# topling/toplingdb

Measured on NVIDIA H100. Metric: compaction_input_kv_MB_per_s, higher is better.
Workload: dtype u8

## Files before the change

### toplingdb_b200/csrc/api.cu

```cuda
#include <cuda_runtime.h>
#include <stdio.h>
#include <stdlib.h>
#include <string.h>

#include <algorithm>
#include <map>
#include <memory>
#include <mutex>
#include <unordered_map>
#include <string>
#include <thread>
#include <vector>

#include "../../include/b200c.h"
#include "inflate_rules.h"
#include "kernels.h"
#include "range_plan.h"
#include "scan.cuh"
#include "sst_host.h"

using namespace b200c;

namespace {

// ... 185 lines not shown
  const char* name;
  cudaEvent_t a, b;
  float us;
};

}

struct b200c_job {
  b200c_params p;
  std::vector<uint64_t> snapshots, fct;
  std::string cf_name, db_id, db_session_id, db_host_id;
  std::vector<Input> inputs;
  std::vector<Output> outputs;
  b200c_stats stats;
  bool ran = false;
  int stage_done = 0;
  int sms = 132;
  cudaStream_t st = nullptr;
  cudaStream_t st2 = nullptr;
  cudaStream_t st_up = nullptr;
  cudaEvent_t ev[5] = {nullptr, nullptr, nullptr, nullptr, nullptr};
  cudaEvent_t evx[4] = {nullptr, nullptr, nullptr, nullptr};
  DevBuf files_d, blk_off, blk_size, blk_state, scan_tmp, run_start, small;
  DevBuf dec[4], mrg[4], splits, tile_state, snaps_d;
  DevBuf esz, eshared, tstat, nxt, disk, rows, tstate, grows, gstate, gflag, gsync, idx_contrib, idx_contrib_off, blocks, files_rec, idx_esz, idx_eoff, idx_sep, out_buf, out_base_d;
  uint64_t n_total = 0, n_out = 0, nblk_in = 0, nblocks_out = 0;
  uint32_t nfiles_out = 0, nruns = 0;
  DevBuf bloom_contrib, bloom_contrib_off;
  DevBuf bloom_hashes;
  DevBuf kv_arena, kv_offs, kv_klens;
  DevBuf run_bounds, run_first_d;
  std::vector<uint64_t> run_start_h;
  HostBuf host_out;
  std::vector<GpKey> gp_small, gp_large;
  std::vector<uint64_t> gp_size;
  std::vector<uint8_t> gp_same;
  DevBuf gp_keys_d, gp_ranks_d, gp_size_d, gp_same_d, gp_cuts_d;
  BoundKey range_lo{}, range_hi{};
  DevBuf clip_d;
  DevBuf cslot, cslot_off, arena;
  std::vector<cudaEvent_t> range_events;
  std::vector<std::string> range_bounds;
  cudaEvent_t wait_ev = nullptr;
  DevBuf vfiles_d, vrun_start;
  HostBuf pin_small, pin_tails, pin_rd, pin_up;
  size_t pin_up_used = 0;
  std::vector<KernelTime> ktimes;
// ... 760 lines not shown
    j->kt_end();
    launches++;
    uint64_t hc[kSmallSlots];
    int rc = read_small(j, small, hc, nullptr, nullptr);
    if (rc) return rc;
    rc = map_dev_err((uint32_t)hc[kSlotErr]);
    if (rc) return rc;
    N_in = hc[kSlotClip];
    range_value_bytes = hc[kSlotClip + 1];
    if (N_in > n_decoded) return fail(B200C_ERR_CUDA, "internal: clipped entry count exceeds the input");
    runs = RunBounds{j->clip_d.as<uint64_t>(), j->clip_d.as<uint64_t>() + K};
    j->stats.num_input_records = N_in;
  }
  return run_merge_encode(j, until, decc, runs, n_decoded, N_in, clipped, range_value_bytes, small, err, launches);
}

int run_merge_encode(b200c_job* j, int until, KeyCols decc, RunBounds runs, uint64_t n_decoded, uint64_t N, bool clipped,
                     uint64_t range_value_bytes, uint64_t* small, uint32_t* err, uint64_t launches) {
  const b200c_params& P = j->p;
  cudaStream_t st = j->st;
  const size_t k = j->nruns;
  const uint64_t mtiles = (N + kMergeNominal - 1) / kMergeNominal;
  CU(j->splits.reserve(8 * (mtiles + 1) * k));
  CU(j->tile_state.reserve(8 * (mtiles + 1)));
  CU(cudaMemsetAsync(j->tile_state.p, 0, 8 * (mtiles + 1), st));
  CU(j->snaps_d.reserve(8 * (P.num_snapshots + 1)));
  if (P.num_snapshots)
    if (int rc = upload_small(j, j->snaps_d.p, j->snapshots.data(), 8 * P.num_snapshots)) return rc;
  CU(j->mrg[0].reserve(16 * (N + 1)));
  CU(j->mrg[1].reserve(8 * (N + 1)));
  CU(j->mrg[2].reserve(8 * (N + 1)));
  CU(j->mrg[3].reserve(4 * (N + 1)));
  CU(j->esz.reserve(4 * (N + 1)));
  CU(j->eshared.reserve(N + 1));
  CU(j->tstat.reserve(sizeof(TileStat) * (mtiles + 2)));
  KeyColsMut mrg{j->mrg[0].as<ulonglong2>(), j->mrg[1].as<uint64_t>(), j->mrg[2].as<uint64_t>(), j->mrg[3].as<uint32_t>()};
  MergeParams mp;
  mp.nruns = (uint32_t)k;
  mp.bottommost = P.bottommost_level != 0;
  mp.nsnapshots = P.num_snapshots;
  mp.snapshots = j->snaps_d.as<uint64_t>();
  mp.earliest_snapshot = P.num_snapshots ? j->snapshots[0] : kMaxSeq;
  mp.filter = P.compaction_filter;
  mp.ttl = P.ttl;
  mp.now = P.ttl_now;
  mp.write_conflict_snapshot = P.earliest_write_conflict_snapshot != 0 && P.earliest_write_conflict_snapshot < kMaxSeq;
  MergeCounters* counters = reinterpret_cast<MergeCounters*>(small + kSlotCounters);
  EncodeWork W;
  memset(&W, 0, sizeof W);
  W.esz = j->esz.as<uint32_t>();
  W.eshared = j->eshared.as<uint8_t>();
  W.tstat = j->tstat.as<TileStat>();
  W.min_s1 = reinterpret_cast<uint32_t*>(small + kSlotMinS1);
  W.totals = small + kSlotTotals;
  if (N) {
    j->kt_begin("merge.partition");
    launch_merge_partition(decc, runs, (uint32_t)k, N, mtiles, j->splits.as<uint64_t>(), err, j->sms, st);
    j->kt_end();
    const MergeSizes msz{W.esz, W.eshared, W.tstat, W.min_s1};
    W.tprefix = j->tile_state.as<unsigned long long>();
    W.nstat = mtiles;
    j->kt_begin("merge.tiles");
    launch_merge_tiles(decc, runs, mp, N, mtiles, j->splits.as<uint64_t>(),
                       j->tile_state.as<unsigned long long>(), reinterpret_cast<uint32_t*>(small + kSlotTicket), mrg, counters, msz, err, st);
    j->kt_end();
    j->kt_begin("merge.sizes_fix");
    launch_merge_sizes_fix(KeyCols{mrg.pfx, mrg.tr, mrg.vref, mrg.meta, 0}, j->tile_state.as<unsigned long long>(), mtiles, msz, st);
    j->kt_end();
    launches += 3;
  }
  CU(cudaEventRecord(j->ev[2], st));
  KeyCols mcols{mrg.pfx, mrg.tr, mrg.vref, mrg.meta, 0};
  uint64_t h[kSmallSlots];
  {
    int rc = read_small(j, small, h, nullptr, nullptr);
    if (rc) return rc;
    rc = map_dev_err((uint32_t)h[kSlotErr]);
    if (rc) return rc;
  }
  if (clipped ? h[kSlotTotalIn] > n_decoded : h[kSlotTotalIn] != n_decoded)
    return fail(B200C_ERR_CORRUPTION, "decoded entry count differs from rocksdb.num.entries");
  MergeCounters mc;
  memcpy(&mc, h + kSlotCounters, sizeof mc);
  const uint64_t n_out = mc.n_out;
  j->n_out = n_out;
  mcols.n = n_out;
// ... 413 lines not shown
  Output& o = j->outputs[i];
  if (cap < o.meta.file_size) return fail(B200C_ERR_INVALID_ARGUMENT, "destination too small");
  if (j->p.output_mem == B200C_MEM_HOST) {
    memcpy(dst, j->host_out.p + o.host_off, o.meta.file_size);
    return B200C_OK;
  }
  CU(cudaSetDevice(j->p.device));
  CU(cudaMemcpy(dst, j->out_buf.as<uint8_t>() + o.dev_off, o.meta.file_size, cudaMemcpyDefault));
  return B200C_OK;
}
int b200c_job_get_stats(const b200c_job* j, b200c_stats* s) {
  if (!j || !s) return fail(B200C_ERR_INVALID_ARGUMENT, "null argument");
  *s = j->stats;
  return B200C_OK;
}
void b200c_job_destroy(b200c_job* j) {
  if (!j) return;
  cudaSetDevice(j->p.device);
  if (j->st) cudaStreamSynchronize(j->st);
  if (j->st2) cudaStreamSynchronize(j->st2);
  if (j->st_up) cudaStreamSynchronize(j->st_up);
  DevBuf* all[] = {&j->files_d, &j->blk_off, &j->blk_size, &j->blk_state, &j->scan_tmp, &j->run_start, &j->run_bounds, &j->run_first_d, &j->kv_arena, &j->kv_offs, &j->kv_klens, &j->bloom_contrib, &j->bloom_contrib_off, &j->bloom_hashes, &j->small,
                   &j->dec[0], &j->dec[1], &j->dec[2], &j->dec[3], &j->mrg[0], &j->mrg[1], &j->mrg[2], &j->mrg[3], &j->splits,
                   &j->tile_state, &j->snaps_d, &j->esz, &j->eshared, &j->tstat, &j->nxt, &j->disk, &j->rows, &j->tstate, &j->grows, &j->gstate, &j->gflag, &j->gsync, &j->idx_contrib, &j->idx_contrib_off, &j->blocks,
                   &j->files_rec, &j->idx_esz, &j->idx_eoff, &j->idx_sep, &j->out_buf, &j->out_base_d};
  for (DevBuf* b : all) b->release();
  j->gp_keys_d.release();
  j->gp_ranks_d.release();
  j->gp_size_d.release();
  j->gp_same_d.release();
  j->gp_cuts_d.release();
  j->clip_d.release();
  j->vfiles_d.release();
  j->vrun_start.release();
  j->cslot.release();
  j->cslot_off.release();
  j->arena.release();
  for (cudaEvent_t e : j->range_events)
    if (e) cudaEventDestroy(e);
  for (auto& in : j->inputs) {
    in.staged.release();
    in.index_inflated.release();
    if (in.up_ev) cudaEventDestroy(in.up_ev);
  }
  if (j->st_up) cudaStreamDestroy(j->st_up);
  j->host_out.release();
  j->pin_small.release();
// ... 167 lines not shown
```

### toplingdb_b200/csrc/kernels.h

```cpp
#pragma once
#include <cuda_runtime.h>
#include <stdint.h>

#include <atomic>

#include "common.cuh"
#include "gp_rules.h"

namespace b200c {

struct PerDeviceFlag {
  std::atomic<uint64_t> mask{0};
  uint64_t bit_of_current_device() const {
    int d = 0;
    cudaGetDevice(&d);
    return 1ull << (d & 63);
  }
  bool is_set(uint64_t bit) const { return (mask.load(std::memory_order_acquire) & bit) != 0; }
  void set(uint64_t bit) { mask.fetch_or(bit, std::memory_order_release); }
};

struct FileDesc {
  const uint8_t* base;
  uint64_t len;
// ... 46 lines not shown
struct MergeParams {
  uint32_t nruns;
  uint32_t bottommost;
  uint32_t nsnapshots;
  const uint64_t* snapshots;
  uint64_t earliest_snapshot;
  uint32_t filter;
  int32_t ttl;
  int64_t now;
  uint32_t write_conflict_snapshot;
};
struct TileStat {
  uint64_t raw_key, raw_value, deletions, smallest_seq, largest_seq;
};
struct MergeSizes {
  uint32_t* esz;
  uint8_t* eshared;
  TileStat* tstat;
  uint32_t* min_s1;
};
struct MergeCounters {
  unsigned long long n_out, n_input_deletions, n_hidden, n_obsolete, raw_key_bytes, raw_value_bytes, n_silent, n_user_drop;
};
struct RunBounds {
  const uint64_t* begin;
  const uint64_t* end;
};
void launch_clip_runs(KeyCols in, RunBounds runs, uint32_t nruns, BoundKey start, uint32_t has_start, BoundKey end,
                      uint32_t has_end, uint64_t* clip, unsigned long long* totals, cudaStream_t st);
void launch_run_bounds(KeyCols in, const uint64_t* file_start, const uint32_t* run_first, uint32_t nruns, uint64_t* bounds, uint32_t* err,
                       cudaStream_t st);
void launch_merge_partition(KeyCols in, RunBounds runs, uint32_t nruns, uint64_t n_total, uint64_t ntiles,
                            uint64_t* splits, uint32_t* err, int sms, cudaStream_t st);
void launch_merge_tiles(KeyCols in, RunBounds runs, MergeParams mp, uint64_t n_total, uint64_t ntiles,
                        const uint64_t* splits, unsigned long long* tile_state, uint32_t* ticket, KeyColsMut out,
                        MergeCounters* counters, MergeSizes ms, uint32_t* err, cudaStream_t st);
void launch_merge_sizes_fix(KeyCols merged, const unsigned long long* tile_state, uint64_t ntiles, MergeSizes ms, cudaStream_t st);

struct GpCut {
  uint64_t entry;
  uint64_t block_bytes;
};
struct EncodeParams {
  uint32_t block_size, block_size_limit , restart_interval;
  uint32_t checksum, format_version, output_level;
  uint64_t max_output_file_size;
  GpCtx gp;
  GpCut* gp_cuts;
  uint32_t* gp_ncuts;
};
using GpKey = BoundKey;
void launch_bloom_count(KeyCols m, uint64_t n, FileRec* files, const uint64_t* nfiles_dev, uint32_t millibits, uint64_t* hashes, int sms, cudaStream_t st);
void launch_bloom_build(const uint64_t* hashes, uint64_t n, const FileRec* files, uint32_t nfiles, uint32_t max_filter_bytes, uint32_t millibits, uint32_t cksum,
                        uint8_t* const* out_base, uint64_t* contrib, const uint64_t* contrib_off, cudaStream_t st);
void launch_gp_ranks(KeyCols m, const GpKey* smallest, const GpKey* largest, uint32_t n, uint64_t* lo, uint64_t* eq, uint64_t* hi,
                     cudaStream_t st);
struct BlockRec {
  uint64_t first_entry;
// ... 83 lines not shown
```

### toplingdb_b200/csrc/merge.cu

```cuda
#include "common.cuh"
#include "group_rules.h"
#include "kernels.h"

namespace b200c {

constexpr int kMT = kMergeTile;
constexpr int kMThreads = 256;
constexpr int kMV = kMT / kMThreads;

__device__ __forceinline__ Key load_key(const KeyCols& c, uint64_t i) {
  Key k;
  ulonglong2 p = c.pfx[i];
  k.hi = p.x;
  k.lo = p.y;
  k.tr = c.tr[i];
  k.ulen = meta_ulen(c.meta[i]);
  return k;
}

__device__ __forceinline__ uint64_t count_before(const KeyCols& c, uint64_t base, uint64_t lo, uint64_t hi, const Key& x,
                                                 bool before_equal) {
  while (lo < hi) {
    uint64_t mid = lo + ((hi - lo) >> 1);
    Key e = load_key(c, base + mid);
    bool precedes = before_equal ? !ikey_less(x, e) : ikey_less(e, x);
    if (precedes) lo = mid + 1;
    else hi = mid;
  }
  return lo;
}

__global__ void __launch_bounds__(128)
merge_partition_kernel(KeyCols in, RunBounds runs, uint32_t nruns, uint64_t n_total, uint64_t ntiles,
                       uint64_t* __restrict__ splits, uint32_t* __restrict__ err) {
  const unsigned lane = threadIdx.x & 31;
  const uint64_t b = (uint64_t)blockIdx.x * (blockDim.x >> 5) + (threadIdx.x >> 5);
  if (b > ntiles) return;
  uint64_t d = b * (uint64_t)kMergeNominal;
  if (d > n_total) d = n_total;
  uint64_t base[2], lo[2], hi[2];
#pragma unroll
  for (int s = 0; s < 2; s++) {
    uint32_t r = lane + 32 * s;
    base[s] = r < nruns ? runs.begin[r] : 0;
    uint64_t n = r < nruns ? runs.end[r] - runs.begin[r] : 0;
    lo[s] = (d == n_total) ? n : 0;
    hi[s] = (d == 0) ? 0 : n;
  }
  for (int guard = 0; guard < 64 * 70; guard++) {
    unsigned long long best = 0;
#pragma unroll
    for (int s = 0; s < 2; s++) {
      unsigned long long wdt = hi[s] - lo[s];
      unsigned long long enc = (wdt << 7) | (unsigned long long)(lane + 32 * s);
      if (wdt && enc > best) best = enc;
    }
#pragma unroll
// ... 18 lines not shown
      sum += c[s];
    }
#pragma unroll
    for (int dd = 16; dd; dd >>= 1) sum += __shfl_xor_sync(0xffffffffu, sum, dd);
    const bool x_before = sum < d;
#pragma unroll
    for (int s = 0; s < 2; s++) {
      uint32_t r = lane + 32 * s;
      if (r >= nruns) continue;
      if (x_before) lo[s] = (r == p) ? m + 1 : c[s];
      else hi[s] = (r == p) ? m : c[s];
    }
  }
  uint64_t tot = lo[0] + lo[1];
#pragma unroll
  for (int dd = 16; dd; dd >>= 1) tot += __shfl_xor_sync(0xffffffffu, tot, dd);
  if (tot != d && lane == 0) atomicOr(err, kErrKeyOrder);
  if (lane == 0 && (*reinterpret_cast<volatile uint32_t*>(err) & (uint32_t)kFlagHasSingleDelete)) atomicOr(err, (uint32_t)kErrGroupTooLong);
#pragma unroll
  for (int s = 0; s < 2; s++) {
    uint32_t r = lane + 32 * s;
    if (r < nruns) splits[b * nruns + r] = lo[s];
  }
}

constexpr uint32_t kPartStride = 64;
struct GroupLanes {
  uint32_t gshift, g, r, sub, gbase, nruns;
};
__device__ __forceinline__ bool entry_precedes(const KeyCols& c, uint64_t i, const Key& x, bool before_equal) {
  const ulonglong2 p = c.pfx[i];
  if (p.x != x.hi) return p.x < x.hi;
  if (p.y != x.lo) return p.y < x.lo;
  const uint32_t ul = meta_ulen(c.meta[i]);
  if (ul != x.ulen) return ul < x.ulen;
  const uint64_t tr = c.tr[i];
  if (tr != x.tr) return tr > x.tr;
  return before_equal;
}
__device__ __forceinline__ void msel_grouped(const KeyCols& in, const GroupLanes& L, uint64_t base, uint64_t stride, uint64_t d, uint64_t& lo,
                                             uint64_t& hi) {
  const uint32_t g = L.g, r = L.r, sub = L.sub, gbase = L.gbase, gshift = L.gshift;
  for (int guard = 0; guard < 64 * 70; guard++) {
    const unsigned long long wdt = hi - lo;
    unsigned long long best = wdt ? ((wdt << 7) | (unsigned long long)r) : 0;
#pragma unroll
// ... 28 lines not shown
      const uint32_t cp = __popc((bal >> gbase) & ((1u << g) - 1u));
      const uint32_t nvalid = w == 0 ? 0 : (w <= g ? (uint32_t)w : g);
      const uint64_t below = __shfl_sync(0xffffffffu, pos, (int)(gbase + (cp ? cp - 1 : 0)));
      const uint64_t above = __shfl_sync(0xffffffffu, pos, (int)(gbase + (cp < g ? cp : g - 1)));
      if (w > 0) {
        if (cp) clo = below + 1;
        if (cp < nvalid) chi = above;
        else if (w <= g) chi = clo;
      }
    }
    const uint64_t c = clo;
    uint64_t sum = sub == 0 ? c : 0;
#pragma unroll
    for (int dd = 16; dd; dd >>= 1) sum += __shfl_xor_sync(0xffffffffu, sum, dd);
    const bool x_before = sum < d;
    if (r < L.nruns) {
      if (x_before) lo = (r == p) ? m + 1 : c;
      else hi = (r == p) ? m : c;
    }
  }
}
__global__ void __launch_bounds__(128, 12)
merge_partition_grouped_kernel(KeyCols in, RunBounds runs, uint32_t nruns, uint32_t gshift, uint64_t n_total,
                               uint64_t ntiles, uint64_t* __restrict__ splits, uint32_t* __restrict__ err, uint32_t chunk) {
  const unsigned lane = threadIdx.x & 31;
  const uint64_t b0 = ((uint64_t)blockIdx.x * (blockDim.x >> 5) + (threadIdx.x >> 5)) * chunk;
  if (b0 > ntiles) return;
  GroupLanes L;
  L.gshift = gshift;
  L.g = 1u << gshift;
  L.r = lane >> gshift;
  L.sub = lane & (L.g - 1);
  L.gbase = L.r << gshift;
  L.nruns = nruns;
  const uint32_t r = L.r, sub = L.sub;
  const uint64_t base = r < nruns ? runs.begin[r] : 0;
  const uint64_t nrun = r < nruns ? runs.end[r] - runs.begin[r] : 0;
  uint64_t prev_lo = 0, prev_d = 0;
  const bool sd_mode = (*reinterpret_cast<volatile uint32_t*>(err) & (uint32_t)kFlagHasSingleDelete) != 0;
  for (uint32_t c = 0; c < chunk; c++) {
    const uint64_t b = b0 + c;
    if (b > ntiles) break;
    uint64_t d = b * (uint64_t)kMergeNominal;
    if (d > n_total) d = n_total;
    uint64_t lo = (d == n_total) ? nrun : 0, hi = (d == 0) ? 0 : nrun;
    if (d != 0 && d != n_total) {
      if (c != 0) {
// ... 39 lines not shown
        const bool ohv = __shfl_xor_sync(0xffffffffu, (int)anyh, dd) != 0, otv = __shfl_xor_sync(0xffffffffu, (int)anyt, dd) != 0;
        if (ohv && (!anyh || ukey_cmp(oh.hi, oh.lo, oh.ulen, mh.hi, mh.lo, mh.ulen) < 0)) mh = oh, anyh = true;
        if (otv && (!anyt || ukey_cmp(ot.hi, ot.lo, ot.ulen, mt.hi, mt.lo, mt.ulen) > 0)) mt = ot, anyt = true;
      }
      if (anyh && anyt && ukey_cmp(mh.hi, mh.lo, mh.ulen, mt.hi, mt.lo, mt.ulen) == 0) {
        uint32_t adv = 0;
        if (r < nruns && sub == 0) {
          while (lo < nrun && adv <= (uint32_t)kSdSpill) {
            const ulonglong2 p = in.pfx[base + lo];
            if (p.x != mh.hi || p.y != mh.lo || meta_ulen(in.meta[base + lo]) != mh.ulen) break;
            lo++;
            adv++;
          }
        }
        uint32_t tadv = adv;
#pragma unroll
        for (int dd = 16; dd; dd >>= 1) tadv += __shfl_xor_sync(0xffffffffu, tadv, dd);
        if (tadv > (uint32_t)kSdSpill && lane == 0) atomicOr(err, (uint32_t)kErrGroupTooLong);
        d += tadv;
        lo = __shfl_sync(0xffffffffu, lo, (int)L.gbase);
      }
    }
    if (r < nruns && sub == 0) splits[b * nruns + r] = lo;
    prev_lo = lo;
    prev_d = d;
  }
}

constexpr uint32_t kSnapCache = 16;
struct TileSmem {
  uint64_t hi[kMT], lo[kMT], tr[kMT];
  uint16_t idx[kMT];
  uint8_t ulen[kMT];
  uint8_t verd[kMT];
  uint32_t seg[kMaxRuns + 1];
  uint32_t lst[2][kMaxRuns + 2];
  uint64_t sbeg[kMaxRuns];
  uint64_t snaps[kSnapCache];
  unsigned long long red[8];
  unsigned long long stat[5];
  uint32_t smin, smax;
  uint32_t wsum[40];
  uint64_t base_out;
  uint32_t tile_id, kept_total;
  Key pred;
  uint32_t has_pred;
};

__device__ __forceinline__ Key skey(const TileSmem& s, uint32_t id) {
  Key k;
  k.hi = s.hi[id];
  k.lo = s.lo[id];
  k.tr = s.tr[id];
  k.ulen = s.ulen[id] & 0x3fu;
  return k;
}
__device__ __forceinline__ uint32_t PH(uint32_t e) { return e ^ ((e >> 4) & 15u); }
__device__ __forceinline__ bool tie_less(const TileSmem& s, uint32_t ib, uint32_t ia) {
  const uint64_t lb = s.lo[ib], la = s.lo[ia];
  if (lb != la) return lb < la;
  const uint32_t ub = s.ulen[ib] & 0x3fu, ua = s.ulen[ia] & 0x3fu;
  if (ub != ua) return ub < ua;
  return s.tr[ib] > s.tr[ia];
}
__device__ __forceinline__ bool id_less(const TileSmem& s, uint32_t ib, uint64_t hb, uint32_t ia, uint64_t ha) {
  if (hb != ha) return hb < ha;
  return tie_less(s, ib, ia);
}

struct PairState {
  uint32_t ai, a1, bi, b1, pend;
};
__device__ __noinline__ void init_pair(const TileSmem& s, const uint32_t* lst, uint32_t nlists, uint32_t o, PairState* ps) {
  uint32_t pi = 0;
  for (;;) {
    uint32_t e = 2 * pi + 2 <= nlists ? lst[2 * pi + 2] : lst[nlists];
    if (o < e) break;
    pi++;
  }
  uint32_t a0 = lst[2 * pi];
  uint32_t a1 = lst[2 * pi + 1];
  bool single = 2 * pi + 1 >= nlists;
  uint32_t b1 = single ? a1 : lst[2 * pi + 2];
  ps->pend = b1;
  ps->a1 = a1;
  ps->b1 = b1;
  if (single) {
    ps->ai = o;
    ps->bi = b1;
    return;
  }
  uint32_t diag = o - a0, an = a1 - a0, bn = b1 - a1;
  uint32_t lo = diag > bn ? diag - bn : 0, hi = diag < an ? diag : an;
  while (lo < hi) {
    uint32_t mid = (lo + hi) >> 1;
    const uint32_t ia = s.idx[PH(a0 + mid)], ib = s.idx[PH(a1 + diag - 1 - mid)];
    if (!id_less(s, ib, s.hi[ib], ia, s.hi[ia])) lo = mid + 1;
    else hi = mid;
  }
  ps->ai = a0 + lo;
  ps->bi = a1 + (diag - lo);
}

__device__ __forceinline__ uint64_t stripe_of(const uint64_t* snaps_s, const uint64_t* snaps_g, uint32_t ns, uint64_t seq,
                                              uint64_t* prev) {
  uint32_t lo = 0, hi = ns;
  while (lo < hi) {
    uint32_t mid = (lo + hi) >> 1;
    uint64_t v = mid < kSnapCache ? snaps_s[mid] : snaps_g[mid];
    if (v < seq) lo = mid + 1;
    else hi = mid;
  }
  *prev = lo == 0 ? 0 : (lo - 1 < kSnapCache ? snaps_s[lo - 1] : snaps_g[lo - 1]);
  return lo < ns ? (lo < kSnapCache ? snaps_s[lo] : snaps_g[lo]) : kMaxSeq;
}

__device__ bool oldest_version_at_most(const KeyCols& in, RunBounds runs, uint32_t nruns, uint64_t hi, uint64_t lo,
                                       uint32_t ulen, uint64_t limit) {
  Key x;
  x.hi = hi;
  x.lo = lo;
  x.ulen = ulen;
  x.tr = 0;
  for (uint32_t r = 0; r < nruns; r++) {
// ... 100 lines not shown
        if (s.seg[mid] <= id0) lo = mid;
        else hi = mid;
      }
      gr.filter_removes_newest = mp.filter == 1 ? (s.ulen[id0] & 0x80u) != 0 : filter_removes(mp, in, s.sbeg[lo] + (id0 - s.seg[lo]));
    }
    gr.first_key_of_the_job = 0;
    GroupVerdict vd[kMaxGroup];
    GroupCounters gc{0, 0, 0, 0};
    if (group_walk(gv, n, gr, vd, &gc) != 0) atomicOr(err, (uint32_t)kErrSingleDelContract);
    for (uint32_t i = 0; i < n; i++)
      s.verd[o + i] = (uint8_t)(0x80u | (vd[i].keep ? 1u : 0u) | (vd[i].zero_seq ? 2u : 0u) | ((vd[i].clear_value & 1u) ? 4u : 0u) |
                                (vd[i].out_type != gv[i].type ? 8u : 0u) | ((vd[i].clear_value & kGrSkipped) ? 16u : 0u));
    *w_hidden += gc.drop_hidden;
    *w_obsolete += gc.drop_obsolete;
    *w_userdrop += gc.drop_user;
  }
  __syncthreads();
}

constexpr int kMergeCtasPerSm = 3;
template <bool kSD>
__global__ void __launch_bounds__(kMThreads, kMergeCtasPerSm)
merge_tiles_kernel(KeyCols in, RunBounds runs, MergeParams mp, uint64_t n_total, uint64_t ntiles,
                   const uint64_t* __restrict__ splits, unsigned long long* tile_state, uint32_t* ticket, KeyColsMut out,
                   MergeCounters* counters, MergeSizes ms, uint32_t* __restrict__ err) {
  extern __shared__ __align__(16) uint8_t smem_raw[];
  TileSmem& s = *reinterpret_cast<TileSmem*>(smem_raw);
  const uint32_t t = threadIdx.x, lane = t & 31, w = t >> 5;
  const uint32_t k = mp.nruns;
  if (((*reinterpret_cast<volatile uint32_t*>(err) & (uint32_t)kFlagHasSingleDelete) != 0) != kSD) return;
  if (t == 0) s.tile_id = atomicAdd(ticket, 1u);
  if (t < 8) s.red[t] = 0;
  if (t < 5) s.stat[t] = t == 3 ? ~0ull : 0ull;
  if (t == 0) {
    s.smin = 0xffffffffu;
    s.smax = 0;
  }
  if (t < kSnapCache && t < mp.nsnapshots) s.snaps[t] = mp.snapshots[t];
  __syncthreads();
  const uint64_t tile = s.tile_id;
  if (tile >= ntiles) return;
  Key* cand = reinterpret_cast<Key*>(s.hi);
  uint32_t* cand_ok = reinterpret_cast<uint32_t*>(s.idx);
  if (t < k) {
    const uint64_t s0 = splits[tile * k + t], s1 = splits[(tile + 1) * k + t];
    const uint64_t b0 = runs.begin[t] + s0;
    s.sbeg[t] = b0;
    s.lst[1][t] = (uint32_t)(s1 - s0);
    cand_ok[t] = s0 != 0;
    if (s0 != 0) cand[t] = load_key(in, b0 - 1);
  }
  __syncthreads();
  if (t == 0) {
    uint32_t acc = 0;
    for (uint32_t r = 0; r < k; r++) {
      s.seg[r] = acc;
      s.lst[0][r] = acc;
      acc += s.lst[1][r];
    }
    s.seg[k] = acc;
    s.lst[0][k] = acc;
    if (acc > kMT) {
      atomicOr(err, kErrKeyOrder);
      s.seg[k] = 0;
    }
    s.has_pred = 0;
    for (uint32_t r = 0; r < k; r++) {
      if (!cand_ok[r]) continue;
      const Key e = cand[r];
      if (!s.has_pred || ikey_less(s.pred, e)) {
        s.pred = e;
        s.has_pred = 1;
      }
    }
  }
  __syncthreads();
  const uint32_t cnt = s.seg[k];
  bool tile_sd = false;
  {
    ulonglong2 lp[kMV];
    uint64_t ltr[kMV];
    uint32_t lmt[kMV];
    uint32_t lr = 0;
    bool my_sd = false;
#pragma unroll
    for (int j = 0; j < kMV; j++) {
      const uint32_t i = t + j * kMThreads;
      lp[j] = make_ulonglong2(0, 0);
      ltr[j] = 0;
      lmt[j] = 0;
      if (i < cnt) {
        while (i >= s.seg[lr + 1]) lr++;
        const uint64_t src = s.sbeg[lr] + (i - s.seg[lr]);
        lp[j] = in.pfx[src];
        ltr[j] = in.tr[src];
        lmt[j] = in.meta[src];
      }
    }
#pragma unroll
    for (int j = 0; j < kMV; j++) {
      const uint32_t i = t + j * kMThreads;
      if (i < cnt) {
        s.hi[i] = lp[j].x;
        s.lo[i] = lp[j].y;
        s.tr[i] = ltr[j];
        if (kSD) my_sd = my_sd || (ltr[j] & 0xff) == kTypeSingleDeletion;
        s.ulen[i] = (uint8_t)(meta_ulen(lmt[j]) | (meta_vlen(lmt[j]) == 0 ? 0x80u : 0u));
        s.idx[PH(i)] = (uint16_t)i;
      }
    }
    if (kSD) tile_sd = __syncthreads_or(my_sd) != 0;
    else __syncthreads();
  }
  uint32_t nlists = k;
  int cur = 0;
  while (nlists > 1) {
    const uint32_t* lst = s.lst[cur];
    uint16_t rid[kMV];
    const uint32_t o0 = t * kMV;
    PairState ps;
    ps.pend = 0;
    ps.ai = ps.a1 = ps.bi = ps.b1 = 0;
    uint32_t ia = 0, ib = 0;
    uint64_t ha = 0, hb = 0;
    bool va = false, vb = false;
#pragma unroll
    for (int x = 0; x < kMV; x++) {
      uint32_t o = o0 + x;
      rid[x] = 0;
      if (o < cnt) {
        if (o >= ps.pend) {
          init_pair(s, lst, nlists, o, &ps);
          va = ps.ai < ps.a1;
          vb = ps.bi < ps.b1;
          if (va) {
            ia = s.idx[PH(ps.ai)];
            ha = s.hi[ia];
          }
          if (vb) {
            ib = s.idx[PH(ps.bi)];
            hb = s.hi[ib];
          }
        }
        const bool take_a = !vb || (va && !id_less(s, ib, hb, ia, ha));
        rid[x] = (uint16_t)(take_a ? ia : ib);
        if (take_a) {
          ps.ai++;
          va = ps.ai < ps.a1;
          if (va) {
            ia = s.idx[PH(ps.ai)];
            ha = s.hi[ia];
          }
        } else {
          ps.bi++;
          vb = ps.bi < ps.b1;
// ... 167 lines not shown
  uint32_t rank = s.wsum[w] + inc - nkeep;
  const uint32_t kept_total = s.kept_total;
  const unsigned long long kAgg = 1ull << 62, kPre = 2ull << 62, kVal = (1ull << 62) - 1;
  if (t == 0) atomicExch(&tile_state[tile], (tile == 0 ? kPre : kAgg) | kept_total);
#pragma unroll
  for (int x = 0; x < kMV; x++) {
    uint32_t o = t * kMV + x;
    if (o < cnt && ((keep_mask >> (16 + x)) & 1)) {
      c_vbytes += meta_vlen(in.meta[col_of(oid[x])]);
    }
  }
  __syncthreads();
#pragma unroll
  for (int x = 0; x < kMV; x++) {
    if ((keep_mask >> x) & 1) {
      s.idx[PH(rank)] = oid[x];
      s.tr[oid[x]] = otr[x];
      if ((keep_mask >> (24 + x)) & 1) s.ulen[oid[x]] |= 0x40u;
      rank++;
    }
  }
  __syncthreads();
  {
    uint64_t gv[kMV];
    uint32_t gm[kMV];
    uint16_t gp[kMV];
#pragma unroll
    for (int j = 0; j < kMV; j++) {
      const uint32_t i = t + j * kMThreads;
      gv[j] = 0;
      gm[j] = 0;
      gp[j] = 0;
      if (i < kept_total) {
        const uint32_t pos = s.idx[PH(i)];
        const uint64_t src = col_of(pos);
        gp[j] = (uint16_t)pos;
        gv[j] = in.vref[src];
        gm[j] = in.meta[src];
        if (s.ulen[pos] & 0x40u) gm[j] = make_meta(meta_ulen(gm[j]), 0);
      }
    }
    if (w == 0) {
      uint64_t base = 0;
      if (tile != 0) {
        int64_t look = (int64_t)tile - 1;
        while (true) {
          const int64_t idx = look - lane;
          unsigned long long sv = kPre;
          if (idx >= 0) {
            sv = *((volatile unsigned long long*)&tile_state[idx]);
            while ((sv >> 62) == 0) {
              __nanosleep(64);
              sv = *((volatile unsigned long long*)&tile_state[idx]);
            }
          }
          const unsigned pre_mask = __ballot_sync(0xffffffffu, (sv >> 62) == 2);
          const int first_pre = pre_mask ? __ffs(pre_mask) - 1 : 32;
          uint64_t contrib = ((int)lane <= first_pre) ? (sv & kVal) : 0;
#pragma unroll
          for (int dd = 16; dd; dd >>= 1) contrib += __shfl_xor_sync(0xffffffffu, contrib, dd);
          base += contrib;
          if (pre_mask) break;
          look -= 32;
        }
        if (lane == 0) atomicExch(&tile_state[tile], kPre | (base + kept_total));
      }
      if (lane == 0) s.base_out = base;
    }
    __syncthreads();
    const uint64_t base_out = s.base_out;
    uint32_t st_kb = 0, st_nd = 0, mn = 0xffffffffu, mx = 0;
    unsigned long long st_vb = 0, st_smin = ~0ull, st_smax = 0;
#pragma unroll
    for (int j = 0; j < kMV; j++) {
      const uint32_t i = t + j * kMThreads;
      if (i < kept_total) {
        const uint32_t pos = gp[j];
        const uint64_t dst = base_out + i;
        const uint64_t chi = s.hi[pos], clo = s.lo[pos], ctr = s.tr[pos];
        const uint32_t cul = s.ulen[pos] & 0x3fu, vlen = meta_vlen(gm[j]);
        out.pfx[dst] = make_ulonglong2(chi, clo);
        out.tr[dst] = ctr;
        out.vref[dst] = gv[j];
        out.meta[dst] = gm[j];
        if (i > 0) {
          const uint32_t pp = s.idx[PH(i - 1)];
          const uint32_t sh = shared_prefix(chi, clo, cul, ctr, s.hi[pp], s.lo[pp], s.ulen[pp] & 0x3fu, s.tr[pp]);
          const uint32_t s1 = entry_size(sh, cul + 8, vlen);
          ms.esz[dst] = s1;
          ms.eshared[dst] = (uint8_t)sh;
          mn = s1 < mn ? s1 : mn;
          mx = s1 > mx ? s1 : mx;
        }
        st_kb += cul + 8;
        st_vb += vlen;
        st_nd += is_deletion_type((uint32_t)(ctr & 0xff));
        const unsigned long long sq = ctr >> 8;
        st_smin = sq < st_smin ? sq : st_smin;
        st_smax = sq > st_smax ? sq : st_smax;
      }
    }
    const unsigned kb = __reduce_add_sync(0xffffffffu, st_kb), nd = __reduce_add_sync(0xffffffffu, st_nd);
    mn = __reduce_min_sync(0xffffffffu, mn);
    mx = __reduce_max_sync(0xffffffffu, mx);
#pragma unroll
    for (int dd = 16; dd; dd >>= 1) {
// ... 110 lines not shown
}
void launch_clip_runs(KeyCols in, RunBounds runs, uint32_t nruns, BoundKey start, uint32_t has_start, BoundKey end,
                      uint32_t has_end, uint64_t* clip, unsigned long long* totals, cudaStream_t st) {
  if (nruns) clip_runs_kernel<<<dim3(kClipSlices, nruns), 256, 0, st>>>(in, runs, nruns, start, has_start, end, has_end, clip, totals);
}
__global__ void run_bounds_kernel(KeyCols in, const uint64_t* __restrict__ file_start, const uint32_t* __restrict__ run_first, uint32_t nruns,
                                  uint64_t* __restrict__ bounds, uint32_t* __restrict__ err) {
  const uint32_t r = blockIdx.x * blockDim.x + threadIdx.x;
  if (r >= nruns) return;
  const uint32_t f0 = run_first[r], f1 = run_first[r + 1];
  bounds[r] = file_start[f0];
  bounds[nruns + r] = file_start[f1];
  for (uint32_t f = f0 + 1; f < f1; f++) {
    const uint64_t e = file_start[f];
    if (e > file_start[f0] && e < file_start[f1] && !ikey_less(load_key(in, e - 1), load_key(in, e))) atomicOr(err, (uint32_t)kErrKeyOrder);
  }
}
void launch_run_bounds(KeyCols in, const uint64_t* file_start, const uint32_t* run_first, uint32_t nruns, uint64_t* bounds, uint32_t* err,
                       cudaStream_t st) {
  if (nruns) run_bounds_kernel<<<(nruns + 63) / 64, 64, 0, st>>>(in, file_start, run_first, nruns, bounds, err);
}

void launch_merge_partition(KeyCols in, RunBounds runs, uint32_t nruns, uint64_t n_total, uint64_t ntiles,
                            uint64_t* splits, uint32_t* err, int sms, cudaStream_t st) {
  unsigned warps = (unsigned)(ntiles + 1);
  if (nruns <= 16) {
    uint32_t kp2 = 2;
    while (kp2 < nruns) kp2 <<= 1;
    uint32_t gshift = 0;
    while ((kp2 << (gshift + 1)) <= 32) gshift++;
    const unsigned wave = (unsigned)sms * 48u;
    uint32_t chunk = (uint32_t)((warps + wave - 1) / wave);
    if (chunk > 4) chunk = 4;
    if (chunk < 1) chunk = 1;
    const unsigned chunks = (warps + chunk - 1) / chunk;
    merge_partition_grouped_kernel<<<(chunks + 3) / 4, 128, 0, st>>>(in, runs, nruns, gshift, n_total, ntiles, splits, err, chunk);
    return;
  }
  merge_partition_kernel<<<(warps + 3) / 4, 128, 0, st>>>(in, runs, nruns, n_total, ntiles, splits, err);
}
static_assert(sizeof(Key) * kMaxRuns <= sizeof(uint64_t) * kMT && 4 * kMaxRuns <= 2 * kMT, "candidate staging must fit");
static_assert(kMergeCtasPerSm * (sizeof(TileSmem) + 1024) <= 227 * 1024, "merge tile must fit three CTAs per SM");
void launch_merge_tiles(KeyCols in, RunBounds runs, MergeParams mp, uint64_t n_total, uint64_t ntiles,
                        const uint64_t* splits, unsigned long long* tile_state, uint32_t* ticket, KeyColsMut out,
                        MergeCounters* counters, MergeSizes ms, uint32_t* err, cudaStream_t st) {
  if (ntiles == 0) return;
  static PerDeviceFlag attr;
  const uint64_t dev_bit = attr.bit_of_current_device();
  if (!attr.is_set(dev_bit)) {
    cudaFuncSetAttribute(merge_tiles_kernel<false>, cudaFuncAttributeMaxDynamicSharedMemorySize, (int)sizeof(TileSmem));
    cudaFuncSetAttribute(merge_tiles_kernel<true>, cudaFuncAttributeMaxDynamicSharedMemorySize, (int)sizeof(TileSmem));
    attr.set(dev_bit);
  }
  merge_tiles_kernel<false><<<(unsigned)ntiles, kMThreads, sizeof(TileSmem), st>>>(in, runs, mp, n_total, ntiles, splits, tile_state, ticket,
                                                                                   out, counters, ms, err);
  merge_tiles_kernel<true><<<(unsigned)ntiles, kMThreads, sizeof(TileSmem), st>>>(in, runs, mp, n_total, ntiles, splits, tile_state, ticket,
                                                                                  out, counters, ms, err);
}
void launch_merge_sizes_fix(KeyCols merged, const unsigned long long* tile_state, uint64_t ntiles, MergeSizes ms, cudaStream_t st) {
  if (ntiles) merge_sizes_fix_kernel<<<(unsigned)((ntiles + 127) / 128), 128, 0, st>>>(merged, tile_state, ntiles, ms);
}

}
```

Before: 244,100.

## Precompute tile predecessor keys in partition and stage tile inputs via cp.async

The partition kernels now compute each tile's predecessor key with a warp shuffle reduction and store it in a new per-tile buffer. This removes the serial loop over runs that thread 0 ran in every merge tile. Merge tiles load keys, tags and value refs straight into shared memory with cp.async, and value refs are now read from shared memory at output time instead of gathered again from global memory. Pair initialisation is partly inlined. Together these add a vref array to shared memory, which may reduce occupancy, and add extra key loads to the partition kernels.

```diff
diff --git a/toplingdb_b200/csrc/api.cu b/toplingdb_b200/csrc/api.cu
--- a/toplingdb_b200/csrc/api.cu
+++ b/toplingdb_b200/csrc/api.cu
@@ -231,7 +231,7 @@
   cudaEvent_t ev[5] = {nullptr, nullptr, nullptr, nullptr, nullptr};
   cudaEvent_t evx[4] = {nullptr, nullptr, nullptr, nullptr};
   DevBuf files_d, blk_off, blk_size, blk_state, scan_tmp, run_start, small;
-  DevBuf dec[4], mrg[4], splits, tile_state, snaps_d;
+  DevBuf dec[4], mrg[4], splits, preds, tile_state, snaps_d;
   DevBuf esz, eshared, tstat, nxt, disk, rows, tstate, grows, gstate, gflag, gsync, idx_contrib, idx_contrib_off, blocks, files_rec, idx_esz, idx_eoff, idx_sep, out_buf, out_base_d;
   uint64_t n_total = 0, n_out = 0, nblk_in = 0, nblocks_out = 0;
   uint32_t nfiles_out = 0, nruns = 0;
@@ -1038,6 +1038,7 @@
   const size_t k = j->nruns;
   const uint64_t mtiles = (N + kMergeNominal - 1) / kMergeNominal;
   CU(j->splits.reserve(8 * (mtiles + 1) * k));
+  CU(j->preds.reserve(sizeof(TilePred) * (mtiles + 1)));
   CU(j->tile_state.reserve(8 * (mtiles + 1)));
   CU(cudaMemsetAsync(j->tile_state.p, 0, 8 * (mtiles + 1), st));
   CU(j->snaps_d.reserve(8 * (P.num_snapshots + 1)));
@@ -1071,13 +1072,13 @@
   W.totals = small + kSlotTotals;
   if (N) {
     j->kt_begin("merge.partition");
-    launch_merge_partition(decc, runs, (uint32_t)k, N, mtiles, j->splits.as<uint64_t>(), err, j->sms, st);
+    launch_merge_partition(decc, runs, (uint32_t)k, N, mtiles, j->splits.as<uint64_t>(), j->preds.as<TilePred>(), err, j->sms, st);
     j->kt_end();
     const MergeSizes msz{W.esz, W.eshared, W.tstat, W.min_s1};
     W.tprefix = j->tile_state.as<unsigned long long>();
     W.nstat = mtiles;
     j->kt_begin("merge.tiles");
-    launch_merge_tiles(decc, runs, mp, N, mtiles, j->splits.as<uint64_t>(),
+    launch_merge_tiles(decc, runs, mp, N, mtiles, j->splits.as<uint64_t>(), j->preds.as<TilePred>(),
                        j->tile_state.as<unsigned long long>(), reinterpret_cast<uint32_t*>(small + kSlotTicket), mrg, counters, msz, err, st);
     j->kt_end();
     j->kt_begin("merge.sizes_fix");
@@ -1537,7 +1538,7 @@
   if (j->st_up) cudaStreamSynchronize(j->st_up);
   DevBuf* all[] = {&j->files_d, &j->blk_off, &j->blk_size, &j->blk_state, &j->scan_tmp, &j->run_start, &j->run_bounds, &j->run_first_d, &j->kv_arena, &j->kv_offs, &j->kv_klens, &j->bloom_contrib, &j->bloom_contrib_off, &j->bloom_hashes, &j->small,
                    &j->dec[0], &j->dec[1], &j->dec[2], &j->dec[3], &j->mrg[0], &j->mrg[1], &j->mrg[2], &j->mrg[3], &j->splits,
-                   &j->tile_state, &j->snaps_d, &j->esz, &j->eshared, &j->tstat, &j->nxt, &j->disk, &j->rows, &j->tstate, &j->grows, &j->gstate, &j->gflag, &j->gsync, &j->idx_contrib, &j->idx_contrib_off, &j->blocks,
+                   &j->preds, &j->tile_state, &j->snaps_d, &j->esz, &j->eshared, &j->tstat, &j->nxt, &j->disk, &j->rows, &j->tstate, &j->grows, &j->gstate, &j->gflag, &j->gsync, &j->idx_contrib, &j->idx_contrib_off, &j->blocks,
                    &j->files_rec, &j->idx_esz, &j->idx_eoff, &j->idx_sep, &j->out_buf, &j->out_base_d};
   for (DevBuf* b : all) b->release();
   j->gp_keys_d.release();
diff --git a/toplingdb_b200/csrc/kernels.h b/toplingdb_b200/csrc/kernels.h
--- a/toplingdb_b200/csrc/kernels.h
+++ b/toplingdb_b200/csrc/kernels.h
@@ -92,6 +92,11 @@
 struct MergeCounters {
   unsigned long long n_out, n_input_deletions, n_hidden, n_obsolete, raw_key_bytes, raw_value_bytes, n_silent, n_user_drop;
 };
+struct alignas(16) TilePred {
+  uint64_t hi, lo, tr;
+  uint32_t ulen, has;
+};
+static_assert(sizeof(TilePred) == 32, "one 32-byte slot per boundary");
 struct RunBounds {
   const uint64_t* begin;
   const uint64_t* end;
@@ -101,9 +106,9 @@
 void launch_run_bounds(KeyCols in, const uint64_t* file_start, const uint32_t* run_first, uint32_t nruns, uint64_t* bounds, uint32_t* err,
                        cudaStream_t st);
 void launch_merge_partition(KeyCols in, RunBounds runs, uint32_t nruns, uint64_t n_total, uint64_t ntiles,
-                            uint64_t* splits, uint32_t* err, int sms, cudaStream_t st);
+                            uint64_t* splits, TilePred* preds, uint32_t* err, int sms, cudaStream_t st);
 void launch_merge_tiles(KeyCols in, RunBounds runs, MergeParams mp, uint64_t n_total, uint64_t ntiles,
-                        const uint64_t* splits, unsigned long long* tile_state, uint32_t* ticket, KeyColsMut out,
+                        const uint64_t* splits, const TilePred* preds, unsigned long long* tile_state, uint32_t* ticket, KeyColsMut out,
                         MergeCounters* counters, MergeSizes ms, uint32_t* err, cudaStream_t st);
 void launch_merge_sizes_fix(KeyCols merged, const unsigned long long* tile_state, uint64_t ntiles, MergeSizes ms, cudaStream_t st);
 
diff --git a/toplingdb_b200/csrc/merge.cu b/toplingdb_b200/csrc/merge.cu
--- a/toplingdb_b200/csrc/merge.cu
+++ b/toplingdb_b200/csrc/merge.cu
@@ -30,9 +30,21 @@
   return lo;
 }
 
+__device__ __forceinline__ void write_pred(Key m, bool has, TilePred* __restrict__ pred) {
+#pragma unroll
+  for (int dd = 16; dd; dd >>= 1) {
+    Key o;
+    o.hi = __shfl_xor_sync(0xffffffffu, m.hi, dd), o.lo = __shfl_xor_sync(0xffffffffu, m.lo, dd);
+    o.tr = __shfl_xor_sync(0xffffffffu, m.tr, dd), o.ulen = __shfl_xor_sync(0xffffffffu, m.ulen, dd);
+    const bool ohas = __shfl_xor_sync(0xffffffffu, (int)has, dd) != 0;
+    if (ohas && (!has || ikey_less(m, o))) m = o, has = true;
+  }
+  if ((threadIdx.x & 31) == 0) *pred = TilePred{m.hi, m.lo, m.tr, m.ulen, has ? 1u : 0u};
+}
+
 __global__ void __launch_bounds__(128)
 merge_partition_kernel(KeyCols in, RunBounds runs, uint32_t nruns, uint64_t n_total, uint64_t ntiles,
-                       uint64_t* __restrict__ splits, uint32_t* __restrict__ err) {
+                       uint64_t* __restrict__ splits, TilePred* __restrict__ preds, uint32_t* __restrict__ err) {
   const unsigned lane = threadIdx.x & 31;
   const uint64_t b = (uint64_t)blockIdx.x * (blockDim.x >> 5) + (threadIdx.x >> 5);
   if (b > ntiles) return;
@@ -97,6 +109,16 @@
     uint32_t r = lane + 32 * s;
     if (r < nruns) splits[b * nruns + r] = lo[s];
   }
+  Key e[2];
+  bool has[2];
+#pragma unroll
+  for (int s = 0; s < 2; s++) {
+    has[s] = lane + 32 * s < nruns && lo[s] > 0;
+    e[s] = Key{0, 0, 0, 0};
+    if (has[s]) e[s] = load_key(in, base[s] + lo[s] - 1);
+  }
+  if (has[1] && (!has[0] || ikey_less(e[0], e[1]))) e[0] = e[1], has[0] = true;
+  write_pred(e[0], has[0], preds + b);
 }
 
 constexpr uint32_t kPartStride = 64;
@@ -171,7 +193,8 @@
 }
 __global__ void __launch_bounds__(128, 12)
 merge_partition_grouped_kernel(KeyCols in, RunBounds runs, uint32_t nruns, uint32_t gshift, uint64_t n_total,
-                               uint64_t ntiles, uint64_t* __restrict__ splits, uint32_t* __restrict__ err, uint32_t chunk) {
+                               uint64_t ntiles, uint64_t* __restrict__ splits, TilePred* __restrict__ preds, uint32_t* __restrict__ err,
+                               uint32_t chunk) {
   const unsigned lane = threadIdx.x & 31;
   const uint64_t b0 = ((uint64_t)blockIdx.x * (blockDim.x >> 5) + (threadIdx.x >> 5)) * chunk;
   if (b0 > ntiles) return;
@@ -257,6 +280,10 @@
       }
     }
     if (r < nruns && sub == 0) splits[b * nruns + r] = lo;
+    const bool has = r < nruns && sub == 0 && lo > 0;
+    Key e{0, 0, 0, 0};
+    if (has) e = load_key(in, base + lo - 1);
+    write_pred(e, has, preds + b);
     prev_lo = lo;
     prev_d = d;
   }
@@ -265,6 +292,7 @@
 constexpr uint32_t kSnapCache = 16;
 struct TileSmem {
   uint64_t hi[kMT], lo[kMT], tr[kMT];
+  uint64_t vref[kMT];
   uint16_t idx[kMT];
   uint8_t ulen[kMT];
   uint8_t verd[kMT];
@@ -282,6 +310,11 @@
   uint32_t has_pred;
 };
 
+__device__ __forceinline__ void cp_async8(void* smem, const void* gmem) {
+  asm volatile("cp.async.ca.shared.global [%0], [%1], 8;" ::"r"((uint32_t)__cvta_generic_to_shared(smem)), "l"(gmem) : "memory");
+}
+__device__ __forceinline__ void cp_async_wait_all() { asm volatile("cp.async.commit_group;\n\tcp.async.wait_group 0;" ::: "memory"); }
+
 __device__ __forceinline__ Key skey(const TileSmem& s, uint32_t id) {
   Key k;
   k.hi = s.hi[id];
@@ -306,7 +339,9 @@
 struct PairState {
   uint32_t ai, a1, bi, b1, pend;
 };
-__device__ __noinline__ void init_pair(const TileSmem& s, const uint32_t* lst, uint32_t nlists, uint32_t o, PairState* ps) {
+__device__ __forceinline__ PairState pair_at(const TileSmem& s, const uint32_t* lst, uint32_t nlists, uint32_t o) {
+  PairState st;
+  PairState* ps = &st;
   uint32_t pi = 0;
   for (;;) {
     uint32_t e = 2 * pi + 2 <= nlists ? lst[2 * pi + 2] : lst[nlists];
@@ -323,7 +358,7 @@
   if (single) {
     ps->ai = o;
     ps->bi = b1;
-    return;
+    return st;
   }
   uint32_t diag = o - a0, an = a1 - a0, bn = b1 - a1;
   uint32_t lo = diag > bn ? diag - bn : 0, hi = diag < an ? diag : an;
@@ -335,6 +370,10 @@
   }
   ps->ai = a0 + lo;
   ps->bi = a1 + (diag - lo);
+  return st;
+}
+__device__ __noinline__ PairState pair_at_call(const TileSmem& s, const uint32_t* lst, uint32_t nlists, uint32_t o) {
+  return pair_at(s, lst, nlists, o);
 }
 
 __device__ __forceinline__ uint64_t stripe_of(const uint64_t* snaps_s, const uint64_t* snaps_g, uint32_t ns, uint64_t seq,
@@ -481,8 +520,8 @@
 template <bool kSD>
 __global__ void __launch_bounds__(kMThreads, kMergeCtasPerSm)
 merge_tiles_kernel(KeyCols in, RunBounds runs, MergeParams mp, uint64_t n_total, uint64_t ntiles,
-                   const uint64_t* __restrict__ splits, unsigned long long* tile_state, uint32_t* ticket, KeyColsMut out,
-                   MergeCounters* counters, MergeSizes ms, uint32_t* __restrict__ err) {
+                   const uint64_t* __restrict__ splits, const TilePred* __restrict__ preds, unsigned long long* tile_state, uint32_t* ticket,
+                   KeyColsMut out, MergeCounters* counters, MergeSizes ms, uint32_t* __restrict__ err) {
   extern __shared__ __align__(16) uint8_t smem_raw[];
   TileSmem& s = *reinterpret_cast<TileSmem*>(smem_raw);
   const uint32_t t = threadIdx.x, lane = t & 31, w = t >> 5;
@@ -499,15 +538,14 @@
   __syncthreads();
   const uint64_t tile = s.tile_id;
   if (tile >= ntiles) return;
-  Key* cand = reinterpret_cast<Key*>(s.hi);
-  uint32_t* cand_ok = reinterpret_cast<uint32_t*>(s.idx);
   if (t < k) {
     const uint64_t s0 = splits[tile * k + t], s1 = splits[(tile + 1) * k + t];
-    const uint64_t b0 = runs.begin[t] + s0;
-    s.sbeg[t] = b0;
+    s.sbeg[t] = runs.begin[t] + s0;
     s.lst[1][t] = (uint32_t)(s1 - s0);
-    cand_ok[t] = s0 != 0;
-    if (s0 != 0) cand[t] = load_key(in, b0 - 1);
+  } else if (t == kMThreads - 1) {
+    const TilePred p = preds[tile];
+    s.pred = Key{p.hi, p.lo, p.tr, p.ulen};
+    s.has_pred = p.has;
   }
   __syncthreads();
   if (t == 0) {
@@ -523,47 +561,35 @@
       atomicOr(err, kErrKeyOrder);
       s.seg[k] = 0;
     }
-    s.has_pred = 0;
-    for (uint32_t r = 0; r < k; r++) {
-      if (!cand_ok[r]) continue;
-      const Key e = cand[r];
-      if (!s.has_pred || ikey_less(s.pred, e)) {
-        s.pred = e;
-        s.has_pred = 1;
-      }
-    }
   }
   __syncthreads();
   const uint32_t cnt = s.seg[k];
   bool tile_sd = false;
   {
-    ulonglong2 lp[kMV];
-    uint64_t ltr[kMV];
     uint32_t lmt[kMV];
     uint32_t lr = 0;
     bool my_sd = false;
 #pragma unroll
     for (int j = 0; j < kMV; j++) {
       const uint32_t i = t + j * kMThreads;
-      lp[j] = make_ulonglong2(0, 0);
-      ltr[j] = 0;
       lmt[j] = 0;
       if (i < cnt) {
         while (i >= s.seg[lr + 1]) lr++;
         const uint64_t src = s.sbeg[lr] + (i - s.seg[lr]);
-        lp[j] = in.pfx[src];
-        ltr[j] = in.tr[src];
+        const uint64_t* p = reinterpret_cast<const uint64_t*>(in.pfx + src);
+        cp_async8(&s.hi[i], p);
+        cp_async8(&s.lo[i], p + 1);
+        cp_async8(&s.tr[i], in.tr + src);
+        cp_async8(&s.vref[i], in.vref + src);
         lmt[j] = in.meta[src];
       }
     }
+    cp_async_wait_all();
 #pragma unroll
     for (int j = 0; j < kMV; j++) {
       const uint32_t i = t + j * kMThreads;
       if (i < cnt) {
-        s.hi[i] = lp[j].x;
-        s.lo[i] = lp[j].y;
-        s.tr[i] = ltr[j];
-        if (kSD) my_sd = my_sd || (ltr[j] & 0xff) == kTypeSingleDeletion;
+        if (kSD) my_sd = my_sd || (s.tr[i] & 0xff) == kTypeSingleDeletion;
         s.ulen[i] = (uint8_t)(meta_ulen(lmt[j]) | (meta_vlen(lmt[j]) == 0 ? 0x80u : 0u));
         s.idx[PH(i)] = (uint16_t)i;
       }
@@ -589,7 +615,8 @@
       rid[x] = 0;
       if (o < cnt) {
         if (o >= ps.pend) {
-          init_pair(s, lst, nlists, o, &ps);
+          if (x == 0) ps = pair_at(s, lst, nlists, o);
+          else ps = pair_at_call(s, lst, nlists, o);
           va = ps.ai < ps.a1;
           vb = ps.bi < ps.b1;
           if (va) {
@@ -803,21 +830,17 @@
   }
   __syncthreads();
   {
-    uint64_t gv[kMV];
     uint32_t gm[kMV];
     uint16_t gp[kMV];
 #pragma unroll
     for (int j = 0; j < kMV; j++) {
       const uint32_t i = t + j * kMThreads;
-      gv[j] = 0;
       gm[j] = 0;
       gp[j] = 0;
       if (i < kept_total) {
         const uint32_t pos = s.idx[PH(i)];
-        const uint64_t src = col_of(pos);
         gp[j] = (uint16_t)pos;
-        gv[j] = in.vref[src];
-        gm[j] = in.meta[src];
+        gm[j] = in.meta[col_of(pos)];
         if (s.ulen[pos] & 0x40u) gm[j] = make_meta(meta_ulen(gm[j]), 0);
       }
     }
@@ -862,7 +885,7 @@
         const uint32_t cul = s.ulen[pos] & 0x3fu, vlen = meta_vlen(gm[j]);
         out.pfx[dst] = make_ulonglong2(chi, clo);
         out.tr[dst] = ctr;
-        out.vref[dst] = gv[j];
+        out.vref[dst] = s.vref[pos];
         out.meta[dst] = gm[j];
         if (i > 0) {
           const uint32_t pp = s.idx[PH(i - 1)];
@@ -1019,7 +1042,7 @@
 }
 
 void launch_merge_partition(KeyCols in, RunBounds runs, uint32_t nruns, uint64_t n_total, uint64_t ntiles,
-                            uint64_t* splits, uint32_t* err, int sms, cudaStream_t st) {
+                            uint64_t* splits, TilePred* preds, uint32_t* err, int sms, cudaStream_t st) {
   unsigned warps = (unsigned)(ntiles + 1);
   if (nruns <= 16) {
     uint32_t kp2 = 2;
@@ -1031,15 +1054,14 @@
     if (chunk > 4) chunk = 4;
     if (chunk < 1) chunk = 1;
     const unsigned chunks = (warps + chunk - 1) / chunk;
-    merge_partition_grouped_kernel<<<(chunks + 3) / 4, 128, 0, st>>>(in, runs, nruns, gshift, n_total, ntiles, splits, err, chunk);
+    merge_partition_grouped_kernel<<<(chunks + 3) / 4, 128, 0, st>>>(in, runs, nruns, gshift, n_total, ntiles, splits, preds, err, chunk);
     return;
   }
-  merge_partition_kernel<<<(warps + 3) / 4, 128, 0, st>>>(in, runs, nruns, n_total, ntiles, splits, err);
-}
-static_assert(sizeof(Key) * kMaxRuns <= sizeof(uint64_t) * kMT && 4 * kMaxRuns <= 2 * kMT, "candidate staging must fit");
+  merge_partition_kernel<<<(warps + 3) / 4, 128, 0, st>>>(in, runs, nruns, n_total, ntiles, splits, preds, err);
+}
 static_assert(kMergeCtasPerSm * (sizeof(TileSmem) + 1024) <= 227 * 1024, "merge tile must fit three CTAs per SM");
 void launch_merge_tiles(KeyCols in, RunBounds runs, MergeParams mp, uint64_t n_total, uint64_t ntiles,
-                        const uint64_t* splits, unsigned long long* tile_state, uint32_t* ticket, KeyColsMut out,
+                        const uint64_t* splits, const TilePred* preds, unsigned long long* tile_state, uint32_t* ticket, KeyColsMut out,
                         MergeCounters* counters, MergeSizes ms, uint32_t* err, cudaStream_t st) {
   if (ntiles == 0) return;
   static PerDeviceFlag attr;
@@ -1049,10 +1071,10 @@
     cudaFuncSetAttribute(merge_tiles_kernel<true>, cudaFuncAttributeMaxDynamicSharedMemorySize, (int)sizeof(TileSmem));
     attr.set(dev_bit);
   }
-  merge_tiles_kernel<false><<<(unsigned)ntiles, kMThreads, sizeof(TileSmem), st>>>(in, runs, mp, n_total, ntiles, splits, tile_state, ticket,
-                                                                                   out, counters, ms, err);
-  merge_tiles_kernel<true><<<(unsigned)ntiles, kMThreads, sizeof(TileSmem), st>>>(in, runs, mp, n_total, ntiles, splits, tile_state, ticket,
-                                                                                  out, counters, ms, err);
+  merge_tiles_kernel<false><<<(unsigned)ntiles, kMThreads, sizeof(TileSmem), st>>>(in, runs, mp, n_total, ntiles, splits, preds, tile_state,
+                                                                                   ticket, out, counters, ms, err);
+  merge_tiles_kernel<true><<<(unsigned)ntiles, kMThreads, sizeof(TileSmem), st>>>(in, runs, mp, n_total, ntiles, splits, preds, tile_state,
+                                                                                  ticket, out, counters, ms, err);
 }
 void launch_merge_sizes_fix(KeyCols merged, const unsigned long long* tile_state, uint64_t ntiles, MergeSizes ms, cudaStream_t st) {
   if (ntiles) merge_sizes_fix_kernel<<<(unsigned)((ntiles + 127) / 128), 128, 0, st>>>(merged, tile_state, ntiles, ms);
```

Result: no change. 245,600, median of 6 (+0.6%).
